# benjaminrwilson/range-view-3d-detection

Measured on AMD Instinct MI355X. Metric: sweeps/sec (fwd+bwd, 64x2048x5 range image), higher is better.
Workload: dtype bf16

## Files before the change

### range_view_3d_detection_amd/csrc/bnbwd.hip

```cpp
#include <algorithm>
#include <stdlib.h>

#include "common.h"
#include "ewpass.h"

int rv_col_reduce(const float* partial, int rows, int cols, double* scratch, int* groups, hipStream_t st);

#ifndef RV_EW_WG_PER_CU
#define RV_EW_WG_PER_CU 1
#endif

namespace {

constexpr int kPixPerBlock = 512;

struct BnbArgs {
    const bf16_t* dout;
    const bf16_t* out;
    const bf16_t* y;
    const float *scale, *shift, *mean, *invstd, *coef;
    int64_t pixels;
    int c, c8;
    int ld_dout, ld_out, ld_y, ld_dy, ld_dres;
    int flags;
    float* partial;
    bf16_t* dy;
    bf16_t* dres;
};

__device__ __forceinline__ void unpack8(const u32x4 v, float* f) {
#pragma unroll
    for (int j = 0; j < 4; ++j) {
        f[2 * j] = bf_lo(v[j]);
        f[2 * j + 1] = bf_hi(v[j]);
    }
}
__device__ __forceinline__ u32x4 pack8(const float* f) {
    u32x4 v;
#pragma unroll
    for (int j = 0; j < 4; ++j) v[j] = pack_bf2(f[2 * j], f[2 * j + 1]);
    return v;
}

struct BnbLoad {
    u32x4 d, y, o;
};
__device__ __forceinline__ BnbLoad load_px(const BnbArgs& a, int64_t px, int c0) {
    BnbLoad r;
    r.d = *(const u32x4*)(a.dout + px * a.ld_dout + c0);
    r.y = *(const u32x4*)(a.y + px * a.ld_y + c0);
    if (a.out) r.o = *(const u32x4*)(a.out + px * a.ld_out + c0);
    return r;
}
__device__ __forceinline__ void masked_grad(const BnbArgs& a, const BnbLoad& r, const float* sc, const float* sh,
                                            const float* mu, const float* is, float* g, float* xhat) {
    float d[8], yv[8];
    unpack8(r.d, d);
    unpack8(r.y, yv);
    if (a.out) {
        float o[8];
        unpack8(r.o, o);
#pragma unroll
        for (int j = 0; j < 8; ++j) d[j] = o[j] > 0.f ? d[j] : 0.f;
    }
#pragma unroll
    for (int j = 0; j < 8; ++j) {
        if ((a.flags & RV_BNB_RELU_Z) && !(yv[j] * sc[j] + sh[j] > 0.f)) d[j] = 0.f;
        g[j] = d[j];
        xhat[j] = (yv[j] - mu[j]) * is[j];
    }
}

__global__ __launch_bounds__(256, RV_EW_WG_PER_CU) void bn_bwd_reduce_kernel(const BnbArgs a) {
    __shared__ float red[256][17];
    const int tid = threadIdx.x;
    const int lanes_px = 256 / a.c8;
    const int oct = tid % a.c8, pl = tid / a.c8;
    const bool active = pl < lanes_px;
    const int c0 = oct * 8;
    float sc[8], sh[8], mu[8], is[8], s0[8], s1[8];
#pragma unroll
    for (int j = 0; j < 8; ++j) {
        sc[j] = a.scale[c0 + j];
        sh[j] = a.shift[c0 + j];
        mu[j] = a.mean[c0 + j];
        is[j] = a.invstd[c0 + j];
        s0[j] = 0.f;
        s1[j] = 0.f;
    }
    const int64_t p0 = (int64_t)blockIdx.x * kPixPerBlock;
    const int64_t p1 = p0 + kPixPerBlock < a.pixels ? p0 + kPixPerBlock : a.pixels;
    if (active) {
        int64_t px = p0 + pl;
        for (; px + 3 * lanes_px < p1; px += 4 * lanes_px) {
            BnbLoad r[4];
#pragma unroll
            for (int u = 0; u < 4; ++u) r[u] = load_px(a, px + u * lanes_px, c0);
#pragma unroll
            for (int u = 0; u < 4; ++u) {
                float g[8], xh[8];
                masked_grad(a, r[u], sc, sh, mu, is, g, xh);
#pragma unroll
                for (int j = 0; j < 8; ++j) {
                    s0[j] += g[j];
                    s1[j] += g[j] * xh[j];
                }
            }
        }
        for (; px < p1; px += lanes_px) {
            float g[8], xh[8];
            masked_grad(a, load_px(a, px, c0), sc, sh, mu, is, g, xh);
#pragma unroll
            for (int j = 0; j < 8; ++j) {
                s0[j] += g[j];
                s1[j] += g[j] * xh[j];
            }
        }
    }
#pragma unroll
    for (int j = 0; j < 8; ++j) {
        red[tid][j] = s0[j];
        red[tid][8 + j] = s1[j];
    }
    __syncthreads();
    for (int i = tid; i < a.c8 * 16; i += 256) {
        const int o = i / 16, j = i - o * 16;
        float s = 0.f;
        for (int l = 0; l < lanes_px; ++l) s += red[l * a.c8 + o][j];
        const int ch = o * 8 + (j & 7);
        a.partial[((int64_t)blockIdx.x * 2 + (j >> 3)) * a.c + ch] = s;
    }
}

struct Bnb2Args {
    const bf16_t *dout, *out, *ya, *yb;
    const float *mean_a, *invstd_a, *mean_b, *invstd_b;
    int64_t pixels;
    int c, c8, ld_dout, ld_out, ld_ya, ld_yb;
    float *partial_a, *partial_b;
};
__global__ __launch_bounds__(256, RV_EW_WG_PER_CU) void bn_bwd_reduce2_kernel(const Bnb2Args a) {
    __shared__ float red[256][25];
    const int tid = threadIdx.x;
    const int lanes_px = 256 / a.c8;
    const int oct = tid % a.c8, pl = tid / a.c8;
    const bool active = pl < lanes_px;
    const int c0 = oct * 8;
    float mua[8], isa[8], mub[8], isb[8], s0[8], sa[8], sb[8];
#pragma unroll
    for (int j = 0; j < 8; ++j) {
        mua[j] = a.mean_a[c0 + j];
        isa[j] = a.invstd_a[c0 + j];
        mub[j] = a.mean_b[c0 + j];
        isb[j] = a.invstd_b[c0 + j];
// ... 296 lines not shown
    constexpr int U = 8;
    const int tid = threadIdx.x;
    const int c4 = a.c8 * 2;
    const int lanes_px = 256 / c4;
    const int quad = tid % c4, pl = tid / c4;
    const int c0 = quad * 4;
    float sc[4], sh[4], mu[4], is[4], s0[4], s1[4];
#pragma unroll
    for (int j = 0; j < 4; ++j) {
        sc[j] = a.scale[c0 + j];
        sh[j] = a.shift[c0 + j];
        mu[j] = a.mean[c0 + j];
        is[j] = a.invstd[c0 + j];
        s0[j] = 0.f;
        s1[j] = 0.f;
    }
    const bool relu_z = (a.flags & RV_BNB_RELU_Z) != 0;
    const int64_t p0 = (int64_t)blockIdx.x * kPixPerBlock;
    const int64_t p1 = p0 + kPixPerBlock < a.pixels ? p0 + kPixPerBlock : a.pixels;
    const int64_t first = p0 + pl;
    const int n_px = (pl < lanes_px && first < p1) ? (int)((p1 - first + lanes_px - 1) / lanes_px) : 0;
    uint32_t o_d = (uint32_t)((first * a.ld_dout + c0) * 2), o_y = (uint32_t)((first * a.ld_y + c0) * 2),
             o_o = OUT ? (uint32_t)((first * a.ld_out + c0) * 2) : 0u;
    const uint32_t s_d = lanes_px * a.ld_dout * 2, s_y = lanes_px * a.ld_y * 2, s_o = lanes_px * a.ld_out * 2;
    auto add = [&](const u32x2 dv, const u32x2 yv, const u32x2 ov) {
#pragma unroll
        for (int h = 0; h < 2; ++h)
#pragma unroll
            for (int e = 0; e < 2; ++e) {
                const int j = 2 * h + e;
                float g = e ? bf_hi(dv[h]) : bf_lo(dv[h]);
                const float y = e ? bf_hi(yv[h]) : bf_lo(yv[h]);
                if (OUT && !((e ? bf_hi(ov[h]) : bf_lo(ov[h])) > 0.f)) g = 0.f;
                if (relu_z && !(y * sc[j] + sh[j] > 0.f)) g = 0.f;
                s0[j] += g;
                s1[j] = fmaf(g, (y - mu[j]) * is[j], s1[j]);
            }
    };
    int i = 0;
    for (; i + U <= n_px; i += U) {
        u32x2 dv[U], yv[U], ov[U];
#pragma unroll
        for (int u = 0; u < U; ++u) {
            dv[u] = ldq(a.dout, o_d + u * s_d);
            yv[u] = ldq(a.y, o_y + u * s_y);
            ov[u] = OUT ? ldq(a.out, o_o + u * s_o) : u32x2{0, 0};
        }
#pragma unroll
        for (int u = 0; u < U; ++u) add(dv[u], yv[u], ov[u]);
        o_d += U * s_d, o_y += U * s_y, o_o += U * s_o;
    }
    for (; i < n_px; ++i) {
        add(ldq(a.dout, o_d), ldq(a.y, o_y), OUT ? ldq(a.out, o_o) : u32x2{0, 0});
        o_d += s_d, o_y += s_y, o_o += s_o;
    }
#pragma unroll
    for (int j = 0; j < 4; ++j) {
        red[tid][j] = s0[j];
        red[tid][4 + j] = s1[j];
    }
    __syncthreads();
    for (int k = tid; k < c4 * 8; k += 256) {
        const int q = k >> 3, j = k & 7;
        float sum = 0.f;
        for (int l = 0; l < lanes_px; ++l) sum += red[l * c4 + q][j];
        a.partial[((int64_t)blockIdx.x * 2 + (j >> 2)) * a.c + q * 4 + (j & 3)] = sum;
    }
}

__global__ __launch_bounds__(256, 5) void bn_bwd_reduce2_lean_kernel(const Bnb2Args a) {
    __shared__ float red[256][13];
    constexpr int U = 4;
    const int tid = threadIdx.x;
    const int c4 = a.c8 * 2;
    const int lanes_px = 256 / c4;
    const int quad = tid % c4, pl = tid / c4;
    const int c0 = quad * 4;
    float mua[4], isa[4], mub[4], isb[4], s0[4], sa[4], sb[4];
#pragma unroll
    for (int j = 0; j < 4; ++j) {
        mua[j] = a.mean_a[c0 + j];
        isa[j] = a.invstd_a[c0 + j];
        mub[j] = a.mean_b[c0 + j];
        isb[j] = a.invstd_b[c0 + j];
        s0[j] = sa[j] = sb[j] = 0.f;
    }
    const int64_t p0 = (int64_t)blockIdx.x * kPixPerBlock;
    const int64_t p1 = p0 + kPixPerBlock < a.pixels ? p0 + kPixPerBlock : a.pixels;
    const int64_t first = p0 + pl;
    const int n_px = (pl < lanes_px && first < p1) ? (int)((p1 - first + lanes_px - 1) / lanes_px) : 0;
    uint32_t o_d = (uint32_t)((first * a.ld_dout + c0) * 2), o_o = (uint32_t)((first * a.ld_out + c0) * 2),
             o_a = (uint32_t)((first * a.ld_ya + c0) * 2), o_b = (uint32_t)((first * a.ld_yb + c0) * 2);
    const uint32_t s_d = lanes_px * a.ld_dout * 2, s_o = lanes_px * a.ld_out * 2, s_a = lanes_px * a.ld_ya * 2, s_b = lanes_px * a.ld_yb * 2;
    auto add = [&](const u32x2 dv, const u32x2 ov, const u32x2 av, const u32x2 bv) {
#pragma unroll
        for (int h = 0; h < 2; ++h)
#pragma unroll
            for (int e = 0; e < 2; ++e) {
                const int j = 2 * h + e;
                const float g = (e ? bf_hi(ov[h]) : bf_lo(ov[h])) > 0.f ? (e ? bf_hi(dv[h]) : bf_lo(dv[h])) : 0.f;
                s0[j] += g;
                sa[j] = fmaf(g, ((e ? bf_hi(av[h]) : bf_lo(av[h])) - mua[j]) * isa[j], sa[j]);
                sb[j] = fmaf(g, ((e ? bf_hi(bv[h]) : bf_lo(bv[h])) - mub[j]) * isb[j], sb[j]);
            }
    };
    int i = 0;
    for (; i + U <= n_px; i += U) {
        u32x2 dv[U], ov[U], av[U], bv[U];
#pragma unroll
        for (int u = 0; u < U; ++u) {
            dv[u] = ldq(a.dout, o_d + u * s_d);
            ov[u] = ldq(a.out, o_o + u * s_o);
            av[u] = ldq(a.ya, o_a + u * s_a);
            bv[u] = ldq(a.yb, o_b + u * s_b);
        }
#pragma unroll
        for (int u = 0; u < U; ++u) add(dv[u], ov[u], av[u], bv[u]);
        o_d += U * s_d, o_o += U * s_o, o_a += U * s_a, o_b += U * s_b;
    }
    for (; i < n_px; ++i) {
        add(ldq(a.dout, o_d), ldq(a.out, o_o), ldq(a.ya, o_a), ldq(a.yb, o_b));
        o_d += s_d, o_o += s_o, o_a += s_a, o_b += s_b;
    }
#pragma unroll
    for (int j = 0; j < 4; ++j) {
        red[tid][j] = s0[j];
        red[tid][4 + j] = sa[j];
        red[tid][8 + j] = sb[j];
    }
    __syncthreads();
    for (int k = tid; k < c4 * 12; k += 256) {
        const int q = k / 12, j = k - q * 12;
        float sum = 0.f;
        for (int l = 0; l < lanes_px; ++l) sum += red[l * c4 + q][j];
        const int ch = q * 4 + (j & 3);
        if (j < 4) {
            a.partial_a[((int64_t)blockIdx.x * 2) * a.c + ch] = sum;
            a.partial_b[((int64_t)blockIdx.x * 2) * a.c + ch] = sum;
        } else if (j < 8) {
            a.partial_a[((int64_t)blockIdx.x * 2 + 1) * a.c + ch] = sum;
        } else {
            a.partial_b[((int64_t)blockIdx.x * 2 + 1) * a.c + ch] = sum;
        }
    }
}

struct Bnb2Apply {
    const bf16_t *dout, *out, *ya, *yb;
    const float *mean_a, *invstd_a, *coef_a, *mean_b, *invstd_b, *coef_b;
    bf16_t *dya, *dyb;
    int64_t pixels;
    int c, c8, ld_dout, ld_out, ld_ya, ld_yb, ld_dya, ld_dyb;
};
template <int MODE>
__global__ __launch_bounds__(256, RV_EW_WG_PER_CU) void bn_bwd_apply2_kernel(const Bnb2Apply a) {
    const int tid = threadIdx.x;
    const int lanes_px = 256 / a.c8;
    const int oct = tid % a.c8, pl = tid / a.c8;
    if (pl >= lanes_px) return;
    const int c0 = oct * 8;
    float mua[8], isa[8], ka0[8], ka1[8], ka2[8], mub[8], isb[8], kb0[8], kb1[8], kb2[8];
#pragma unroll
    for (int j = 0; j < 8; ++j) {
        mua[j] = a.mean_a[c0 + j], isa[j] = a.invstd_a[c0 + j];
        ka0[j] = a.coef_a[c0 + j], ka1[j] = a.coef_a[a.c + c0 + j], ka2[j] = a.coef_a[2 * a.c + c0 + j];
        mub[j] = a.mean_b[c0 + j], isb[j] = a.invstd_b[c0 + j];
        kb0[j] = a.coef_b[c0 + j], kb1[j] = a.coef_b[a.c + c0 + j], kb2[j] = a.coef_b[2 * a.c + c0 + j];
    }
    const int64_t per = ((a.pixels + gridDim.x - 1) / gridDim.x + lanes_px - 1) / lanes_px * lanes_px;
    const int64_t end = (int64_t)(blockIdx.x + 1) * per < a.pixels ? (int64_t)(blockIdx.x + 1) * per : a.pixels;
    for (int64_t px = (int64_t)blockIdx.x * per + pl; px < end; px += lanes_px) {
        float d[8], o[8], ya[8], yb[8], ra[8], rb[8];
        unpack8(ld16<MODE>(a.dout + px * a.ld_dout + c0), d);
        unpack8(ld16<MODE>(a.out + px * a.ld_out + c0), o);
        unpack8(ld16<MODE>(a.ya + px * a.ld_ya + c0), ya);
        unpack8(ld16<MODE>(a.yb + px * a.ld_yb + c0), yb);
#pragma unroll
        for (int j = 0; j < 8; ++j) {
            const float g = o[j] > 0.f ? d[j] : 0.f;
            const float xa = (ya[j] - mua[j]) * isa[j], xb = (yb[j] - mub[j]) * isb[j];
            ra[j] = ka0[j] * (g - ka1[j] - xa * ka2[j]);
            rb[j] = kb0[j] * (g - kb1[j] - xb * kb2[j]);
        }
        st16<MODE>(a.dya + px * a.ld_dya + c0, pack8(ra));
        st16<MODE>(a.dyb + px * a.ld_dyb + c0, pack8(rb));
    }
}

__global__ __launch_bounds__(256) void ew_mask_grad_kernel(int64_t pixels, int c8, const bf16_t* dout, int ld_dout,
                                                           const bf16_t* out, int ld_out, bf16_t* d, int ld_d,
                                                           int accumulate) {
    const int64_t total = pixels * c8;
    for (int64_t i = blockIdx.x * (int64_t)blockDim.x + threadIdx.x; i < total; i += (int64_t)gridDim.x * blockDim.x) {
        const int64_t px = i / c8;
        const int c0 = (int)(i - px * c8) * 8;
        float g[8];
        unpack8(*(const u32x4*)(dout + px * ld_dout + c0), g);
        if (out) {
            float o[8];
            unpack8(*(const u32x4*)(out + px * ld_out + c0), o);
#pragma unroll
            for (int j = 0; j < 8; ++j) g[j] = o[j] > 0.f ? g[j] : 0.f;
        }
        bf16_t* p = d + px * ld_d + c0;
        if (accumulate) {
            float old[8];
            unpack8(*(const u32x4*)p, old);
#pragma unroll
            for (int j = 0; j < 8; ++j) g[j] += old[j];
        }
        *(u32x4*)p = pack8(g);
    }
}

template <int CIN, bool RECOMP>
__global__ __launch_bounds__(256) void bn_bwd_smallk_reduce_kernel(const BnbArgs a, const bf16_t* v, int ld_v, const bf16_t* w, int ld_w) {
    __shared__ float red[256][9];
    const int tid = threadIdx.x;
    const int lanes_px = 256 / a.c8;
    const int oct = tid % a.c8, pl = tid / a.c8;
    const bool active = pl < lanes_px;
    const int c0 = oct * 8;
    float sc[8], sh[8], mu[8], is[8], s0[8], s1[8], r[CIN][8], wt[RECOMP ? 8 : 1][CIN];
#pragma unroll
    for (int j = 0; j < 8; ++j) {
        sc[j] = a.scale[c0 + j];
        sh[j] = a.shift[c0 + j];
        mu[j] = a.mean[c0 + j];
        is[j] = a.invstd[c0 + j];
        s0[j] = 0.f;
        s1[j] = 0.f;
#pragma unroll
        for (int d = 0; d < CIN; ++d) r[d][j] = 0.f;
        if (RECOMP) {
#pragma unroll
            for (int e = 0; e < CIN; ++e) wt[RECOMP ? j : 0][e] = bf2f(w[(int64_t)(c0 + j) * ld_w + e]);
        }
    }
    const int64_t p0 = (int64_t)blockIdx.x * kPixPerBlock;
    const int64_t p1 = p0 + kPixPerBlock < a.pixels ? p0 + kPixPerBlock : a.pixels;
    auto load = [&](int64_t px) {
        BnbLoad l;
        l.d = *(const u32x4*)(a.dout + px * a.ld_dout + c0);
        if (!RECOMP) l.y = *(const u32x4*)(a.y + px * a.ld_y + c0);
        if (a.out) l.o = *(const u32x4*)(a.out + px * a.ld_out + c0);
        return l;
    };
    auto accumulate = [&](const BnbLoad& l, const u32x4 wv) {
        float g[8], xh[8], vv[8];
        unpack8(wv, vv);
        if (RECOMP) {
            float d[8];
            unpack8(l.d, d);
            if (a.out) {
                float o[8];
                unpack8(l.o, o);
#pragma unroll
                for (int j = 0; j < 8; ++j) d[j] = o[j] > 0.f ? d[j] : 0.f;
            }
#pragma unroll
            for (int j = 0; j < 8; ++j) {
                float y = 0.f;
#pragma unroll
                for (int e = 0; e < CIN; ++e) y += wt[RECOMP ? j : 0][e] * vv[e];
                if ((a.flags & RV_BNB_RELU_Z) && !(y * sc[j] + sh[j] > 0.f)) d[j] = 0.f;
                g[j] = d[j];
                xh[j] = (y - mu[j]) * is[j];
            }
        } else {
            masked_grad(a, l, sc, sh, mu, is, g, xh);
        }
#pragma unroll
        for (int j = 0; j < 8; ++j) {
            s0[j] += g[j];
            s1[j] += g[j] * xh[j];
#pragma unroll
            for (int d = 0; d < CIN; ++d) r[d][j] += g[j] * vv[d];
        }
    };
    if (active) {
        int64_t px = p0 + pl;
        for (; px + lanes_px < p1; px += 2 * lanes_px) {
            const BnbLoad l0 = load(px), l1 = load(px + lanes_px);
            const u32x4 w0 = *(const u32x4*)(v + px * ld_v), w1 = *(const u32x4*)(v + (px + lanes_px) * ld_v);
            accumulate(l0, w0);
            accumulate(l1, w1);
        }
        for (; px < p1; px += lanes_px) accumulate(load(px), *(const u32x4*)(v + px * ld_v));
    }
    for (int plane = 0; plane < 2 + CIN; ++plane) {
#pragma unroll
        for (int j = 0; j < 8; ++j) {
            float val = plane == 0 ? s0[j] : (plane == 1 ? s1[j] : 0.f);
#pragma unroll
            for (int d = 0; d < CIN; ++d)
                if (plane == 2 + d) val = r[d][j];
            red[tid][j] = val;
        }
        __syncthreads();
        for (int i = tid; i < a.c8 * 8; i += 256) {
            const int o = i >> 3, j = i & 7;
            float s = 0.f;
            for (int l = 0; l < lanes_px; ++l) s += red[l * a.c8 + o][j];
            a.partial[((int64_t)blockIdx.x * (2 + CIN) + plane) * a.c + o * 8 + j] = s;
        }
        __syncthreads();
    }
}

template <int CIN>
__global__ __launch_bounds__(256) void smallk_moments_kernel(const bf16_t* v, int ld_v, int64_t pixels, float* partial) {
    __shared__ float red[256];
    float m[CIN + CIN * CIN];
#pragma unroll
    for (int i = 0; i < CIN + CIN * CIN; ++i) m[i] = 0.f;
    const int64_t per = (pixels + gridDim.x - 1) / gridDim.x;
    const int64_t p0 = blockIdx.x * per, p1 = p0 + per < pixels ? p0 + per : pixels;
    for (int64_t px = p0 + threadIdx.x; px < p1; px += 256) {
        float vv[8];
        unpack8(*(const u32x4*)(v + px * ld_v), vv);
#pragma unroll
        for (int d = 0; d < CIN; ++d) {
            m[d] += vv[d];
#pragma unroll
            for (int e = 0; e < CIN; ++e) m[CIN + d * CIN + e] += vv[d] * vv[e];
        }
    }
    for (int i = 0; i < CIN + CIN * CIN; ++i) {
        red[threadIdx.x] = m[i];
        __syncthreads();
        for (int h = 128; h > 0; h >>= 1) {
            if ((int)threadIdx.x < h) red[threadIdx.x] += red[threadIdx.x + h];
            __syncthreads();
        }
        if (threadIdx.x == 0) partial[(int64_t)blockIdx.x * (CIN + CIN * CIN) + i] = red[0];
        __syncthreads();
    }
}

// ... 107 lines not shown
    for (int i = blockIdx.x * blockDim.x + threadIdx.x; i < cols; i += gridDim.x * blockDim.x) {
        double s = 0.0;
        for (int r = 0; r < n_rows; ++r) s += rows[(int64_t)r * cols + i];
        out[i] = s;
    }
}

int fill(BnbArgs* a, int64_t pixels, int32_t c, const void* dout, int32_t ld_dout, const void* out, int32_t ld_out,
         const void* y, int32_t ld_y, const float* scale, const float* shift, const float* mean, const float* invstd,
         int32_t flags) {
    RV_REQUIRE(dout && (y || (flags & RV_BNB_Y_FROM_INPUT)) && scale && shift && mean && invstd, "bn backward: null argument");
    RV_REQUIRE(c % 8 == 0 && c / 8 <= 256 && ld_dout % 8 == 0 && ld_y % 8 == 0 && (!out || ld_out % 8 == 0), "bn backward: channels / strides must be multiples of 8 (c <= 2048)");
    memset(a, 0, sizeof(*a));
    a->dout = (const bf16_t*)dout;
    a->out = (const bf16_t*)out;
    a->y = (const bf16_t*)y;
    a->scale = scale;
    a->shift = shift;
    a->mean = mean;
    a->invstd = invstd;
    a->pixels = pixels;
    a->c = c;
    a->c8 = c / 8;
    a->ld_dout = ld_dout;
    a->ld_out = ld_out;
    a->ld_y = ld_y;
    a->flags = flags;
    return 0;
}

int check_extent(const char* who, int64_t pixels, int32_t c, int32_t ld_dout, const void* out, int32_t ld_out, const void* y, int32_t ld_y) {
    RV_REQUIRE(pixels > 0 && c > 0 && ld_dout >= c && (!y || ld_y >= c) && (!out || ld_out >= c),
               "%s: empty tensor, or a row pitch below the channel count", who);
    return 0;
}

}

extern "C" int32_t rv_bn_bwd_rows(int64_t pixels) { return (int32_t)((pixels + kPixPerBlock - 1) / kPixPerBlock); }

extern "C" int rv_bn_bwd_reduce(int64_t pixels, int32_t c, const void* dout, int32_t ld_dout, const void* out,
                                int32_t ld_out, const void* y, int32_t ld_y, const float* scale, const float* shift,
                                const float* mean, const float* invstd, int32_t flags, float* partial, rvStream stream) {
    BnbArgs a;
    if (fill(&a, pixels, c, dout, ld_dout, out, ld_out, y, ld_y, scale, shift, mean, invstd, flags)) return 1;
    RV_REQUIRE(partial, "rv_bn_bwd_reduce: null partial buffer");
    if (check_extent("rv_bn_bwd_reduce", pixels, c, ld_dout, out, ld_out, y, ld_y)) return 1;
    a.partial = partial;
    const RvEwPlan plan = rv_plan_bnb_reduce(pixels, c, ld_dout, ld_out, ld_y, out != nullptr);
    if (plan.form == RV_EW_FORM_LEAN) {
        if (out) hipLaunchKernelGGL(bn_bwd_reduce_lean_kernel<true>, dim3(plan.grid), dim3(256), 0, (hipStream_t)stream, a);
        else hipLaunchKernelGGL(bn_bwd_reduce_lean_kernel<false>, dim3(plan.grid), dim3(256), 0, (hipStream_t)stream, a);
        RV_CHECK_LAUNCH("bn_bwd_reduce_lean_kernel");
        return 0;
    }
    hipLaunchKernelGGL(bn_bwd_reduce_kernel, dim3(plan.grid), dim3(256), 0, (hipStream_t)stream, a);
    RV_CHECK_LAUNCH("bn_bwd_reduce_kernel");
    return 0;
}

extern "C" int rv_bn_bwd_reduce_pair(int64_t pixels, int32_t c, const void* dout, int32_t ld_dout, const void* out, int32_t ld_out,
                                     const void* ya, int32_t ld_ya, const float* mean_a, const float* invstd_a, const void* yb, int32_t ld_yb,
                                     const float* mean_b, const float* invstd_b, float* partial_a, float* partial_b, rvStream stream) {
    RV_REQUIRE(dout && out && ya && yb && mean_a && invstd_a && mean_b && invstd_b && partial_a && partial_b, "rv_bn_bwd_reduce_pair: null argument");
    RV_REQUIRE(pixels > 0 && c > 0 && c % 8 == 0 && c <= 2048 && ld_dout % 8 == 0 && ld_out % 8 == 0 && ld_ya % 8 == 0 && ld_yb % 8 == 0 &&
                   ld_dout >= c && ld_out >= c && ld_ya >= c && ld_yb >= c,
               "rv_bn_bwd_reduce_pair: channels / strides must be multiples of 8 (at most 2048 channels)");
    Bnb2Args a{};
    a.dout = (const bf16_t*)dout, a.out = (const bf16_t*)out, a.ya = (const bf16_t*)ya, a.yb = (const bf16_t*)yb;
    a.mean_a = mean_a, a.invstd_a = invstd_a, a.mean_b = mean_b, a.invstd_b = invstd_b;
    a.pixels = pixels, a.c = c, a.c8 = c / 8, a.ld_dout = ld_dout, a.ld_out = ld_out, a.ld_ya = ld_ya, a.ld_yb = ld_yb;
    a.partial_a = partial_a, a.partial_b = partial_b;
    const RvEwPlan plan = rv_plan_bnb_reduce_pair(pixels, c, ld_dout, ld_out, ld_ya, ld_yb);
    if (plan.form == RV_EW_FORM_LEAN) {
        hipLaunchKernelGGL(bn_bwd_reduce2_lean_kernel, dim3(plan.grid), dim3(256), 0, (hipStream_t)stream, a);
        RV_CHECK_LAUNCH("bn_bwd_reduce2_lean_kernel");
        return 0;
    }
    hipLaunchKernelGGL(bn_bwd_reduce2_kernel, dim3(plan.grid), dim3(256), 0, (hipStream_t)stream, a);
    RV_CHECK_LAUNCH("bn_bwd_reduce2_kernel");
    return 0;
}

extern "C" int rv_bn_bwd_finalize(const float* partial, int32_t rows, int32_t c, int64_t count, const float* gamma,
                                  const float* invstd, float* dgamma, float* dbeta, int32_t accumulate, float* coef,
                                  rvStream stream) {
    RV_REQUIRE(partial && gamma && invstd && coef, "rv_bn_bwd_finalize: null argument");
    RV_REQUIRE(count > 0 || (count < 0 && rows == 1), "rv_bn_bwd_finalize: a device-side count (count < 0) needs the single row of all-reduced totals");
    const float* count_dev = count < 0 ? partial + 2 * c : nullptr;
    const RvEwPlan plan = rv_plan_bn_finalize(rows, c);
    if (plan.form == RV_EW_FORM_FUSED_FINALIZE) {
        hipLaunchKernelGGL(bn_bwd_reduce_finalize_kernel, dim3(plan.grid), dim3(256), 0, (hipStream_t)stream, partial, rows, c,
                           1.0 / (double)count, gamma, invstd, dgamma, dbeta, accumulate, coef, count_dev);
        RV_CHECK_LAUNCH("bn_bwd_reduce_finalize_kernel");
        return 0;
    }
    RV_REQUIRE(count > 0, "rv_bn_bwd_finalize: the two-stage path (> 2048 rows) takes a host-side count only");
    double* scratch = (double*)(partial + (int64_t)rows * 2 * c);
    int groups;
    if (rv_col_reduce(partial, rows, 2 * c, scratch, &groups, (hipStream_t)stream)) return 1;
    hipLaunchKernelGGL(bn_bwd_finalize_kernel, dim3(plan.grid), dim3(256), 0, (hipStream_t)stream, scratch, groups, c,
                       1.0 / (double)count, gamma, invstd, dgamma, dbeta, accumulate, coef);
    RV_CHECK_LAUNCH("bn_bwd_finalize_kernel");
    return 0;
}

extern "C" int rv_bn_bwd_apply(int64_t pixels, int32_t c, const void* dout, int32_t ld_dout, const void* out,
                               int32_t ld_out, const void* y, int32_t ld_y, const float* scale, const float* shift,
                               const float* mean, const float* invstd, const float* coef, int32_t flags, void* dy,
                               int32_t ld_dy, void* dres, int32_t ld_dres, rvStream stream) {
    BnbArgs a;
    if (fill(&a, pixels, c, dout, ld_dout, out, ld_out, y, ld_y, scale, shift, mean, invstd, flags)) return 1;
    RV_REQUIRE(coef && dy && ld_dy % 8 == 0 && (!dres || ld_dres % 8 == 0), "rv_bn_bwd_apply: bad outputs");
    if (check_extent("rv_bn_bwd_apply", pixels, c, ld_dout, out, ld_out, y, ld_y)) return 1;
    RV_REQUIRE(ld_dy >= c && (!dres || ld_dres >= c), "rv_bn_bwd_apply: a row pitch below the channel count");
    a.coef = coef;
    a.dy = (bf16_t*)dy;
    a.ld_dy = ld_dy;
    a.dres = (bf16_t*)dres;
    a.ld_dres = ld_dres;
    const RvEwPlan plan = rv_plan_bnb_apply(pixels, c, ld_dout, ld_out, ld_y, ld_dy, ld_dres, out != nullptr, dres != nullptr, flags);
    if (plan.form == RV_EW_FORM_LEAN) {
        using K = void (*)(const BnbArgs);
        static const K table[16] = {bn_bwd_apply_lean_kernel<0>,  bn_bwd_apply_lean_kernel<1>,  bn_bwd_apply_lean_kernel<2>,  bn_bwd_apply_lean_kernel<3>,
                                    bn_bwd_apply_lean_kernel<4>,  bn_bwd_apply_lean_kernel<5>,  bn_bwd_apply_lean_kernel<6>,  bn_bwd_apply_lean_kernel<7>,
                                    bn_bwd_apply_lean_kernel<4>,  bn_bwd_apply_lean_kernel<5>,  bn_bwd_apply_lean_kernel<6>,  bn_bwd_apply_lean_kernel<7>,
                                    bn_bwd_apply_lean_kernel<12>, bn_bwd_apply_lean_kernel<13>, bn_bwd_apply_lean_kernel<14>, bn_bwd_apply_lean_kernel<15>};
        hipLaunchKernelGGL(table[plan.index], dim3(plan.grid), dim3(256), 0, (hipStream_t)stream, a);
        RV_CHECK_LAUNCH("bn_bwd_apply_lean_kernel");
        return 0;
    }
    if (plan.nontemporal)
        hipLaunchKernelGGL(bn_bwd_apply_kernel<1>, dim3(plan.grid), dim3(256), 0, (hipStream_t)stream, a);
    else
        hipLaunchKernelGGL(bn_bwd_apply_kernel<0>, dim3(plan.grid), dim3(256), 0, (hipStream_t)stream, a);
    RV_CHECK_LAUNCH("bn_bwd_apply_kernel");
    return 0;
}

extern "C" int rv_bn_bwd_apply_pair(int64_t pixels, int32_t c, const void* dout, int32_t ld_dout, const void* out, int32_t ld_out,
                                    const void* ya, int32_t ld_ya, const float* mean_a, const float* invstd_a, const float* coef_a, void* dya,
                                    int32_t ld_dya, const void* yb, int32_t ld_yb, const float* mean_b, const float* invstd_b,
                                    const float* coef_b, void* dyb, int32_t ld_dyb, rvStream stream) {
    RV_REQUIRE(dout && out && ya && yb && mean_a && invstd_a && coef_a && dya && mean_b && invstd_b && coef_b && dyb, "rv_bn_bwd_apply_pair: null argument");
    RV_REQUIRE(pixels > 0 && c > 0 && c % 8 == 0 && c <= 2048 && ld_dout % 8 == 0 && ld_out % 8 == 0 && ld_ya % 8 == 0 && ld_yb % 8 == 0 &&
                   ld_dya % 8 == 0 && ld_dyb % 8 == 0 && ld_dout >= c && ld_out >= c && ld_ya >= c && ld_yb >= c && ld_dya >= c && ld_dyb >= c,
               "rv_bn_bwd_apply_pair: channels / strides must be multiples of 8 (at most 2048 channels)");
    Bnb2Apply a{};
    a.dout = (const bf16_t*)dout, a.out = (const bf16_t*)out, a.ya = (const bf16_t*)ya, a.yb = (const bf16_t*)yb;
    a.mean_a = mean_a, a.invstd_a = invstd_a, a.coef_a = coef_a, a.mean_b = mean_b, a.invstd_b = invstd_b, a.coef_b = coef_b;
    a.dya = (bf16_t*)dya, a.dyb = (bf16_t*)dyb;
    a.pixels = pixels, a.c = c, a.c8 = c / 8;
    a.ld_dout = ld_dout, a.ld_out = ld_out, a.ld_ya = ld_ya, a.ld_yb = ld_yb, a.ld_dya = ld_dya, a.ld_dyb = ld_dyb;
    const RvEwPlan plan = rv_plan_bnb_apply_pair(pixels, c);
    if (plan.nontemporal)
        hipLaunchKernelGGL(bn_bwd_apply2_kernel<1>, dim3(plan.grid), dim3(256), 0, (hipStream_t)stream, a);
    else
        hipLaunchKernelGGL(bn_bwd_apply2_kernel<0>, dim3(plan.grid), dim3(256), 0, (hipStream_t)stream, a);
    RV_CHECK_LAUNCH("bn_bwd_apply2_kernel");
    return 0;
}

extern "C" int rv_ew_mask_grad(int64_t pixels, int32_t c, const void* dout, int32_t ld_dout, const void* out,
                               int32_t ld_out, void* d, int32_t ld_d, int32_t accumulate, rvStream stream) {
    RV_REQUIRE(dout && d, "rv_ew_mask_grad: null argument");
    RV_REQUIRE(c % 8 == 0 && ld_dout % 8 == 0 && ld_d % 8 == 0 && (!out || ld_out % 8 == 0), "rv_ew_mask_grad: channels / strides must be multiples of 8");
    RV_REQUIRE(pixels > 0 && c > 0 && ld_dout >= c && ld_d >= c && (!out || ld_out >= c), "rv_ew_mask_grad: empty tensor, or a row pitch below the channel count");
    hipLaunchKernelGGL(ew_mask_grad_kernel, dim3(rv_plan_ew_mask_grad(pixels, c).grid), dim3(256), 0, (hipStream_t)stream, pixels,
                       c / 8, (const bf16_t*)dout, ld_dout, (const bf16_t*)out, ld_out, (bf16_t*)d, ld_d, accumulate);
    RV_CHECK_LAUNCH("ew_mask_grad_kernel");
    return 0;
}

extern "C" int rv_ew_pass_info(int32_t pass, int64_t pixels_or_rows, int32_t c, const int32_t* ld, int32_t has_out, int32_t has_dres,
                               int32_t flags, int32_t* host_info) {
    RV_REQUIRE(host_info, "rv_ew_pass_info: null argument");
    RV_REQUIRE(pixels_or_rows > 0 && c > 0, "rv_ew_pass_info: empty tensor");
    const bool finalize = pass == RV_EW_PASS_BN_FINALIZE || pass == RV_EW_PASS_BWD_FINALIZE;
    RvEwPlan plan;
    if (finalize) {
        RV_REQUIRE(pixels_or_rows <= INT32_MAX, "rv_ew_pass_info: too many partial rows");
        RV_REQUIRE(!flags || pixels_or_rows == 1, "rv_ew_pass_info: a device-side count needs the single row of all-reduced totals");
        plan = rv_plan_bn_finalize((int)pixels_or_rows, c);
        plan.index = flags ? 1 : 0;
    } else {
        RV_REQUIRE(c % 8 == 0, "rv_ew_pass_info: channels must be a multiple of 8");
        const int32_t dense[5] = {c, c, c, c, c};
        if (!ld) ld = dense;
        RV_REQUIRE(c <= 2048 || pass == RV_EW_PASS_COMBINE || pass == RV_EW_PASS_MASK_GRAD, "rv_ew_pass_info: at most 2048 channels");
        switch (pass) {
            case RV_EW_PASS_COMBINE: plan = rv_plan_ew_combine(pixels_or_rows, c, has_out != 0); break;
            case RV_EW_PASS_MASK_GRAD: plan = rv_plan_ew_mask_grad(pixels_or_rows, c); break;
            case RV_EW_PASS_BWD_REDUCE: plan = rv_plan_bnb_reduce(pixels_or_rows, c, ld[0], ld[1], ld[2], has_out != 0); break;
            case RV_EW_PASS_BWD_REDUCE_PAIR: plan = rv_plan_bnb_reduce_pair(pixels_or_rows, c, ld[0], ld[1], ld[2], ld[3]); break;
            case RV_EW_PASS_BWD_APPLY: plan = rv_plan_bnb_apply(pixels_or_rows, c, ld[0], ld[1], ld[2], ld[3], ld[4], has_out != 0, has_dres != 0, flags); break;
            case RV_EW_PASS_BWD_APPLY_PAIR: plan = rv_plan_bnb_apply_pair(pixels_or_rows, c); break;
            default: RV_FAIL("rv_ew_pass_info: unknown pass %d", pass);
        }
    }
    host_info[0] = plan.form;
    host_info[1] = plan.nontemporal;
    host_info[2] = plan.grid;
    host_info[3] = plan.index;
    return 0;
}

extern "C" int64_t rv_bn_bwd_smallk_workspace_bytes(int64_t pixels, int32_t c, int32_t cin) {
    const int CIN = cin <= 4 ? 4 : 8;
    const int64_t rows = rv_bn_bwd_rows(pixels);
    const int64_t planes = 2 + CIN, mcols = CIN + CIN * CIN;
    int64_t bytes = ((rows + 2 * 64) * planes * c + (1024 + 2 * 64) * mcols) * (int64_t)sizeof(float) + 256;
    bytes = (bytes + 7) & ~(int64_t)7;
    return bytes + (planes * c + 80) * 8;
}

extern "C" int rv_bn_bwd_smallk_sums(int64_t pixels, int32_t c, const void* dout, int32_t ld_dout, const void* out, int32_t ld_out,
                                     const void* y, int32_t ld_y, const float* scale, const float* shift, const float* mean,
                                     const float* invstd, int32_t flags, const void* v, int32_t ld_v, int32_t cin, const void* w_packed,
                                     int32_t ld_w, double* sums, double* moms, void* workspace, rvStream stream) {
    BnbArgs a;
    if (fill(&a, pixels, c, dout, ld_dout, out, ld_out, y, ld_y, scale, shift, mean, invstd, flags)) return 1;
    RV_REQUIRE(v && sums && moms && workspace, "rv_bn_bwd_smallk_sums: null argument");
    const bool recomp = (flags & RV_BNB_Y_FROM_INPUT) != 0;
    RV_REQUIRE(!recomp || (w_packed && ld_w >= cin), "rv_bn_bwd_smallk_sums: RV_BNB_Y_FROM_INPUT needs the packed weight");
    const bf16_t* wq = (const bf16_t*)w_packed;
    RV_REQUIRE(cin >= 1 && cin <= 8 && ld_v % 8 == 0 && ld_v >= 8, "rv_bn_bwd_smallk: 1 <= cin <= 8, input rows of at least 8 channels");
    const int CIN = cin <= 4 ? 4 : 8;
    const int rows = rv_bn_bwd_rows(pixels), planes = 2 + CIN, mcols = CIN + CIN * CIN;
    float* part_g = (float*)workspace;
    double* scr_g = (double*)(part_g + (int64_t)rows * planes * c);
    float* part_m = (float*)(scr_g + (int64_t)64 * planes * c);
    const int mblocks = pixels >= 1024 * 256 ? 1024 : (int)((pixels + 255) / 256);
    double* scr_m = (double*)(part_m + (int64_t)1024 * mcols);
    hipStream_t st = (hipStream_t)stream;
    a.partial = part_g;
    if (CIN == 4) {
        if (recomp) hipLaunchKernelGGL((bn_bwd_smallk_reduce_kernel<4, true>), dim3(rows), dim3(256), 0, st, a, (const bf16_t*)v, ld_v, wq, ld_w);
        else hipLaunchKernelGGL((bn_bwd_smallk_reduce_kernel<4, false>), dim3(rows), dim3(256), 0, st, a, (const bf16_t*)v, ld_v, wq, ld_w);
        hipLaunchKernelGGL(smallk_moments_kernel<4>, dim3(mblocks), dim3(256), 0, st, (const bf16_t*)v, ld_v, pixels, part_m);
    } else {
        if (recomp) hipLaunchKernelGGL((bn_bwd_smallk_reduce_kernel<8, true>), dim3(rows), dim3(256), 0, st, a, (const bf16_t*)v, ld_v, wq, ld_w);
        else hipLaunchKernelGGL((bn_bwd_smallk_reduce_kernel<8, false>), dim3(rows), dim3(256), 0, st, a, (const bf16_t*)v, ld_v, wq, ld_w);
        hipLaunchKernelGGL(smallk_moments_kernel<8>, dim3(mblocks), dim3(256), 0, st, (const bf16_t*)v, ld_v, pixels, part_m);
    }
    RV_CHECK_LAUNCH("bn_bwd_smallk reduce kernels");
    int groups_g, groups_m;
    if (rv_col_reduce(part_g, rows, planes * c, scr_g, &groups_g, st)) return 1;
    if (rv_col_reduce(part_m, mblocks, mcols, scr_m, &groups_m, st)) return 1;
    hipLaunchKernelGGL(sum_rows_f64_kernel, dim3(rv_ceil_div(planes * c, 128)), dim3(128), 0, st, scr_g, groups_g, planes * c, sums);
    hipLaunchKernelGGL(sum_rows_f64_kernel, dim3(1), dim3(128), 0, st, scr_m, groups_m, mcols, moms);
    RV_CHECK_LAUNCH("sum_rows_f64_kernel");
    return 0;
}

int rv_pos_bwd_launch(int64_t pixels, const void* dy2, const void* w2_scatter, const void* rel, int32_t ld_rel, int32_t cin,
                      const void* w1_packed, int32_t ld_w1, const float* scale1, const float* shift1, const float* mean1,
                      const float* invstd1, float* partial, int32_t planes, int32_t max_rows, int32_t* rows, int32_t c, hipStream_t stream);

extern "C" int rv_pos_backward_sums(int64_t pixels, int32_t c, const void* dy2, const void* w2_scatter, const void* rel, int32_t ld_rel,
                                    int32_t cin, const void* w1_packed, int32_t ld_w1, const float* scale1, const float* shift1,
                                    const float* mean1, const float* invstd1, double* sums, double* moms, void* workspace,
                                    rvStream stream) {
    RV_REQUIRE(dy2 && w2_scatter && rel && w1_packed && scale1 && shift1 && mean1 && invstd1 && sums && moms && workspace,
               "rv_pos_backward_sums: null argument");
    RV_REQUIRE((c == 256 || c == 128) && cin >= 1 && cin <= 3 && ld_rel % 8 == 0 && ld_rel >= 8 && pixels > 0,
               "rv_pos_backward_sums: built for 256 or 128 channels, cin <= 3");
    const int CIN = 4, planes = 2 + CIN, mcols = CIN + CIN * CIN;
    const int rows_max = rv_bn_bwd_rows(pixels);
    float* part_g = (float*)workspace;
    double* scr_g = (double*)(part_g + (int64_t)rows_max * planes * c);
    float* part_m = (float*)(scr_g + (int64_t)64 * planes * c);
    const int mblocks = pixels >= 1024 * 256 ? 1024 : (int)((pixels + 255) / 256);
    double* scr_m = (double*)(part_m + (int64_t)1024 * mcols);
    hipStream_t st = (hipStream_t)stream;
    int rows = 0;
    if (rv_pos_bwd_launch(pixels, dy2, w2_scatter, rel, ld_rel, cin, w1_packed, ld_w1, scale1, shift1, mean1, invstd1, part_g, planes, rows_max,
                          &rows, c, st))
        return 1;
    hipLaunchKernelGGL(smallk_moments_kernel<4>, dim3(mblocks), dim3(256), 0, st, (const bf16_t*)rel, ld_rel, pixels, part_m);
    RV_CHECK_LAUNCH("smallk_moments_kernel");
    int groups_g, groups_m;
    if (rv_col_reduce(part_g, rows, planes * c, scr_g, &groups_g, st)) return 1;
    if (rv_col_reduce(part_m, mblocks, mcols, scr_m, &groups_m, st)) return 1;
    hipLaunchKernelGGL(sum_rows_f64_kernel, dim3(rv_ceil_div(planes * c, 128)), dim3(128), 0, st, scr_g, groups_g, planes * c, sums);
    hipLaunchKernelGGL(sum_rows_f64_kernel, dim3(1), dim3(128), 0, st, scr_m, groups_m, mcols, moms);
    RV_CHECK_LAUNCH("sum_rows_f64_kernel");
    return 0;
}

extern "C" int rv_bn_bwd_smallk_from_sums(int32_t c, int32_t cin, const double* sums, const double* moms, const double* global_s01,
                                          const void* w_packed, int32_t ld_w, const float* gamma, const float* stat_mean,
                                          const float* stat_invstd, int64_t count, float* dgamma, float* dbeta, float* dW,
                                          rvStream stream) {
    RV_REQUIRE(sums && moms && w_packed && gamma && stat_mean && stat_invstd && dgamma && dbeta && dW, "rv_bn_bwd_smallk_from_sums: null argument");
    RV_REQUIRE(cin >= 1 && cin <= 8 && (count > 0 || global_s01), "rv_bn_bwd_smallk_from_sums: bad shape (count < 0 needs global_s01)");
    hipStream_t st = (hipStream_t)stream;
    const double* count_dev = count < 0 ? global_s01 + 2 * (int64_t)c : nullptr;
    const double inv = count > 0 ? 1.0 / (double)count : 0.0;
    if (cin <= 4)
        hipLaunchKernelGGL(bn_bwd_smallk_finalize_kernel<4>, dim3(rv_ceil_div(c, 64)), dim3(64), 0, st, sums, 1, moms, 1, c, cin, inv,
                           gamma, stat_mean, stat_invstd, (const bf16_t*)w_packed, ld_w, global_s01, count_dev, dgamma, dbeta, dW);
    else
        hipLaunchKernelGGL(bn_bwd_smallk_finalize_kernel<8>, dim3(rv_ceil_div(c, 64)), dim3(64), 0, st, sums, 1, moms, 1, c, cin, inv,
                           gamma, stat_mean, stat_invstd, (const bf16_t*)w_packed, ld_w, global_s01, count_dev, dgamma, dbeta, dW);
    RV_CHECK_LAUNCH("bn_bwd_smallk_finalize_kernel");
    return 0;
}

extern "C" int rv_bn_bwd_smallk(int64_t pixels, int32_t c, const void* dout, int32_t ld_dout, const void* out, int32_t ld_out,
                                const void* y, int32_t ld_y, const float* scale, const float* shift, const float* mean,
                                const float* invstd, int32_t flags, const void* v, int32_t ld_v, int32_t cin, const void* w_packed,
// ... 79 lines not shown
```

Measured before the change: 41.88.

## Stage paired BN-backward coefficients in LDS and unroll apply2 pixel loop

```diff
diff --git a/profiles/overlap_budgeted.py b/profiles/overlap_budgeted.py
--- /dev/null
+++ b/profiles/overlap_budgeted.py
@@ -0,0 +1,21 @@
+import sys
+
+seq, on = [], False
+for ln in open(sys.argv[1]):
+    if ln.startswith("# sequence"):
+        on = True
+        continue
+    if on and ln.strip():
+        s, d, name = ln.split(None, 2)
+        seq.append((float(s), float(d), name.strip()))
+wg = [(s, s + d) for s, d, n in seq if n.startswith("wgrad3_kernel")]
+print(f"# {sys.argv[1]}: wgrad3_kernel {len(wg)} launches, {sum(e - s for s, e in wg):.1f} us in the step")
+tot = {}
+for s, d, n in seq:
+    if not (n.startswith("bn_bwd_apply2_kernel") or n.startswith("meta_bwd_apply_kernel")):
+        continue
+    tot[n] = tot.get(n, 0.0) + d
+    over = [f"wgrad3 {ws:.0f} -> {we:.0f} (shared {min(we, s + d) - max(ws, s):.0f} us)" for ws, we in wg if ws < s + d and we > s]
+    print(f"{n:28s} start {s:9.1f}  {d:8.1f} us   " + ("; ".join(over) if over else "no wgrad3 resident"))
+for n, t in sorted(tot.items()):
+    print(f"# total {n}: {t:.1f} us")
diff --git a/range_view_3d_detection_amd/csrc/bnbwd.hip b/range_view_3d_detection_amd/csrc/bnbwd.hip
--- a/range_view_3d_detection_amd/csrc/bnbwd.hip
+++ b/range_view_3d_detection_amd/csrc/bnbwd.hip
@@ -1,5 +1,6 @@
 #include <algorithm>
 #include <stdlib.h>
+#include <type_traits>
 
 #include "common.h"
 #include "ewpass.h"
@@ -602,39 +603,89 @@
     int64_t pixels;
     int c, c8, ld_dout, ld_out, ld_ya, ld_yb, ld_dya, ld_dyb;
 };
+constexpr int kPairRows = 10, kPairQuads = 2 * kPairRows + 1;
+static inline int rv_pair_table_bytes(int c) { return (c / 8) * kPairQuads * (int)sizeof(f32x4); }
 template <int MODE>
-__global__ __launch_bounds__(256, RV_EW_WG_PER_CU) void bn_bwd_apply2_kernel(const Bnb2Apply a) {
+__global__ __launch_bounds__(256, 5) void bn_bwd_apply2_kernel(const Bnb2Apply a) {
+    extern __shared__ f32x4 pair_tab[];
+    constexpr int U = 2;
     const int tid = threadIdx.x;
-    const int lanes_px = 256 / a.c8;
-    const int oct = tid % a.c8, pl = tid / a.c8;
+    const int c8 = a.c8;
+    for (int ch = tid; ch < a.c; ch += 256) {
+        const float v[kPairRows] = {a.mean_a[ch], a.invstd_a[ch], a.coef_a[ch], a.coef_a[a.c + ch], a.coef_a[2 * a.c + ch],
+                                    a.mean_b[ch], a.invstd_b[ch], a.coef_b[ch], a.coef_b[a.c + ch], a.coef_b[2 * a.c + ch]};
+        float* dst = (float*)pair_tab + ((ch >> 3) * kPairQuads + ((ch >> 2) & 1)) * 4 + (ch & 3);
+#pragma unroll
+        for (int r = 0; r < kPairRows; ++r) dst[r * 8] = v[r];
+    }
+    __syncthreads();
+    const int lanes_px = 256 / c8;
+    const int oct = tid % c8, pl = tid / c8;
     if (pl >= lanes_px) return;
     const int c0 = oct * 8;
-    float mua[8], isa[8], ka0[8], ka1[8], ka2[8], mub[8], isb[8], kb0[8], kb1[8], kb2[8];
-#pragma unroll
-    for (int j = 0; j < 8; ++j) {
-        mua[j] = a.mean_a[c0 + j], isa[j] = a.invstd_a[c0 + j];
-        ka0[j] = a.coef_a[c0 + j], ka1[j] = a.coef_a[a.c + c0 + j], ka2[j] = a.coef_a[2 * a.c + c0 + j];
-        mub[j] = a.mean_b[c0 + j], isb[j] = a.invstd_b[c0 + j];
-        kb0[j] = a.coef_b[c0 + j], kb1[j] = a.coef_b[a.c + c0 + j], kb2[j] = a.coef_b[2 * a.c + c0 + j];
-    }
+    const f32x4* const tab = pair_tab + oct * kPairQuads;
+    const uint32_t t_d = (uint32_t)(pl * a.ld_dout + c0) * 2, t_o = (uint32_t)(pl * a.ld_out + c0) * 2,
+                   t_a = (uint32_t)(pl * a.ld_ya + c0) * 2, t_b = (uint32_t)(pl * a.ld_yb + c0) * 2,
+                   t_da = (uint32_t)(pl * a.ld_dya + c0) * 2, t_db = (uint32_t)(pl * a.ld_dyb + c0) * 2;
+    auto ld = [&](const bf16_t* row, uint32_t off) { return ld16<MODE>((const bf16_t*)((const char*)row + off)); };
+    auto st = [&](bf16_t* row, uint32_t off, const u32x4 v) { st16<MODE>((bf16_t*)((char*)row + off), v); };
+    auto run = [&](int64_t p, auto n_tag) {
+        constexpr int N = decltype(n_tag)::value;
+        uint32_t o_d = t_d, o_o = t_o, o_a = t_a, o_b = t_b, o_da = t_da, o_db = t_db;
+        asm volatile("" : "+v"(o_d), "+v"(o_o), "+v"(o_a), "+v"(o_b), "+v"(o_da), "+v"(o_db)::"memory");
+        u32x4 dv[N], ov[N], av[N], bv[N], ra[N], rb[N];
+#pragma unroll
+        for (int u = 0; u < N; ++u) {
+            const int64_t q = p + u * lanes_px;
+            dv[u] = ld(a.dout + q * a.ld_dout, o_d);
+            ov[u] = ld(a.out + q * a.ld_out, o_o);
+            av[u] = ld(a.ya + q * a.ld_ya, o_a);
+            bv[u] = ld(a.yb + q * a.ld_yb, o_b);
+        }
+#pragma unroll
+        for (int h = 0; h < 2; ++h) {
+            float g[N][4];
+#pragma unroll
+            for (int u = 0; u < N; ++u)
+#pragma unroll
+                for (int e = 0; e < 4; ++e) {
+                    const uint32_t dw = dv[u][2 * h + (e >> 1)], ow = ov[u][2 * h + (e >> 1)];
+                    const float d = (e & 1) ? bf_hi(dw) : bf_lo(dw), o = (e & 1) ? bf_hi(ow) : bf_lo(ow);
+                    g[u][e] = o > 0.f ? d : 0.f;
+                }
+#pragma unroll
+            for (int bn = 0; bn < 2; ++bn) {
+                __builtin_amdgcn_sched_barrier(0);
+                const f32x4* t = tab + bn * kPairRows + h;
+                const f32x4 mu = t[0], is = t[2], k0 = t[4], k1 = t[6], k2 = t[8];
+#pragma unroll
+                for (int u = 0; u < N; ++u) {
+                    float r[4];
+#pragma unroll
+                    for (int e = 0; e < 4; ++e) {
+                        const uint32_t yw = (bn ? bv[u] : av[u])[2 * h + (e >> 1)];
+                        const float y = (e & 1) ? bf_hi(yw) : bf_lo(yw);
+                        const float x = (y - mu[e]) * is[e];
+                        r[e] = k0[e] * (g[u][e] - k1[e] - x * k2[e]);
+                    }
+                    (bn ? rb[u] : ra[u])[2 * h] = pack_bf2(r[0], r[1]);
+                    (bn ? rb[u] : ra[u])[2 * h + 1] = pack_bf2(r[2], r[3]);
+                }
+            }
+        }
+#pragma unroll
+        for (int u = 0; u < N; ++u) {
+            const int64_t q = p + u * lanes_px;
+            st(a.dya + q * a.ld_dya, o_da, ra[u]);
+            st(a.dyb + q * a.ld_dyb, o_db, rb[u]);
+        }
+    };
     const int64_t per = ((a.pixels + gridDim.x - 1) / gridDim.x + lanes_px - 1) / lanes_px * lanes_px;
     const int64_t end = (int64_t)(blockIdx.x + 1) * per < a.pixels ? (int64_t)(blockIdx.x + 1) * per : a.pixels;
-    for (int64_t px = (int64_t)blockIdx.x * per + pl; px < end; px += lanes_px) {
-        float d[8], o[8], ya[8], yb[8], ra[8], rb[8];
-        unpack8(ld16<MODE>(a.dout + px * a.ld_dout + c0), d);
-        unpack8(ld16<MODE>(a.out + px * a.ld_out + c0), o);
-        unpack8(ld16<MODE>(a.ya + px * a.ld_ya + c0), ya);
-        unpack8(ld16<MODE>(a.yb + px * a.ld_yb + c0), yb);
-#pragma unroll
-        for (int j = 0; j < 8; ++j) {
-            const float g = o[j] > 0.f ? d[j] : 0.f;
-            const float xa = (ya[j] - mua[j]) * isa[j], xb = (yb[j] - mub[j]) * isb[j];
-            ra[j] = ka0[j] * (g - ka1[j] - xa * ka2[j]);
-            rb[j] = kb0[j] * (g - kb1[j] - xb * kb2[j]);
-        }
-        st16<MODE>(a.dya + px * a.ld_dya + c0, pack8(ra));
-        st16<MODE>(a.dyb + px * a.ld_dyb + c0, pack8(rb));
-    }
+    int64_t p = (int64_t)blockIdx.x * per;
+    for (; p + U * lanes_px <= end; p += U * lanes_px) run(p, std::integral_constant<int, U>{});
+    for (; p < end; p += lanes_px)
+        if (p + pl < end) run(p, std::integral_constant<int, 1>{});
 }
 
 __global__ __launch_bounds__(256) void ew_mask_grad_kernel(int64_t pixels, int c8, const bf16_t* dout, int ld_dout,
@@ -1048,11 +1099,16 @@
     a.dya = (bf16_t*)dya, a.dyb = (bf16_t*)dyb;
     a.pixels = pixels, a.c = c, a.c8 = c / 8;
     a.ld_dout = ld_dout, a.ld_out = ld_out, a.ld_ya = ld_ya, a.ld_yb = ld_yb, a.ld_dya = ld_dya, a.ld_dyb = ld_dyb;
+    RV_REQUIRE(rv_max_ld(ld_dout, ld_out, ld_ya, ld_yb, std::max(ld_dya, ld_dyb)) < (1 << 23), "rv_bn_bwd_apply_pair: row pitch of 2^23 elements and more");
     const RvEwPlan plan = rv_plan_bnb_apply_pair(pixels, c);
-    if (plan.nontemporal)
-        hipLaunchKernelGGL(bn_bwd_apply2_kernel<1>, dim3(plan.grid), dim3(256), 0, (hipStream_t)stream, a);
-    else
-        hipLaunchKernelGGL(bn_bwd_apply2_kernel<0>, dim3(plan.grid), dim3(256), 0, (hipStream_t)stream, a);
+    const int lds = rv_pair_table_bytes(c);
+    if (plan.nontemporal) {
+        RV_LDS_OPT_IN(rv_pair_table_bytes(2048), bn_bwd_apply2_kernel<1>);
+        hipLaunchKernelGGL(bn_bwd_apply2_kernel<1>, dim3(plan.grid), dim3(256), lds, (hipStream_t)stream, a);
+    } else {
+        RV_LDS_OPT_IN(rv_pair_table_bytes(2048), bn_bwd_apply2_kernel<0>);
+        hipLaunchKernelGGL(bn_bwd_apply2_kernel<0>, dim3(plan.grid), dim3(256), lds, (hipStream_t)stream, a);
+    }
     RV_CHECK_LAUNCH("bn_bwd_apply2_kernel");
     return 0;
 }
```

Result: slower. 41.29 (-1.4%).
